# XUANTIE-RV/csi-nn2

Hardware: AMD Instinct MI355X
Metric: mobilenetv1_int8_images_per_sec (higher is better)
Workload: dtype i8; 1 GPU; mobilenetv1 int8 NHWC batch 1/GPU, 28 conv layers in 15 launches, hipGraph replay via csinn_*; ops_per_image=1137480704, algorithmic_bytes_per_image=8323144, algorithmic_bytes_per_image_survey=14444616, parallelism=replicas x1

## Files before the change

### csi-nn2_amd/csrc/stemdw_fused.hip

```cpp
#include <stdio.h>
#include <stdlib.h>

#include "dw_patch.h"

namespace shl {

struct StemDwArgs {
    ConvArgs st;
    ConvArgs dw;
    int32_t bh, bw;
    int32_t tiles_x, tiles_y;
    int32_t rw, npx;
    uint32_t rw_magic, bw_magic;
};

template <int EPQ, int EPD>
__global__ __launch_bounds__(256) void stemdw_fused_kernel(StemDwArgs f)
{
    extern __shared__ __attribute__((aligned(16))) char smem[];
    const ConvArgs &q = f.st;
    const ConvArgs &d = f.dw;
    asm volatile("" ::"s"(q.in), "s"(q.w), "s"(q.acc_init), "s"(q.mult), "s"(q.bias), "s"(q.H), "s"(q.W), "s"(q.Ho), "s"(q.Wo), "s"(q.sh),
                 "s"(q.sw), "s"(q.pt), "s"(q.pl), "s"(q.dh), "s"(q.dw), "s"(q.in_zp));
    asm volatile("" ::"s"(f.bh), "s"(f.bw), "s"(f.tiles_y), "s"(f.rw), "s"(f.npx), "s"(f.rw_magic), "s"(f.bw_magic), "s"(d.N), "s"(d.sh),
                 "s"(d.sw), "s"(d.pt), "s"(d.pl), "s"(d.w), "s"(d.acc_init), "s"(d.mult), "s"(d.bias), "s"(d.out));
    asm volatile("" ::"s"(q.out_zp), "s"(q.out_zp_f), "s"(q.clamp_lo), "s"(q.clamp_hi), "s"(d.out_zp), "s"(d.out_zp_f), "s"(d.clamp_lo),
                 "s"(d.clamp_hi), "s"(d.in_zp), "s"(d.Ho), "s"(d.Wo), "s"(d.H), "s"(d.W), "s"(d.C));
    const int tid = threadIdx.x;
    int32_t *w_lds = reinterpret_cast<int32_t *>(smem);
    int32_t *t_tab = w_lds + 7 * 32;
    uint32_t *patch = reinterpret_cast<uint32_t *>(t_tab + 96);
    if (tid < 224) w_lds[tid] = static_cast<const int32_t *>(q.w)[tid];
    if (tid < 96) {
        const int which = tid >> 5, i = tid & 31;
        t_tab[tid] = which == 0 ? q.acc_init[i] : which == 1 ? __float_as_int(q.mult[i]) : __float_as_int(q.bias[i]);
    }
    const int tx = blockIdx.x;
    int ty = blockIdx.y, n = 0;
    if (d.N > 1) {
        n = ty / f.tiles_y;
        ty -= n * f.tiles_y;
    }
    const int oy0 = ty * f.bh, ox0 = tx * f.bw;
    const int ry0 = oy0 * d.sh - d.pt, rx0 = ox0 * d.sw - d.pl;
    const DwThreadConsts dwk = dw_load_consts(d, 0, tid);

    const int8_t *img = static_cast<const int8_t *>(q.in) + (int64_t)n * q.H * q.W * 3;
    const int ntasks = 2 * f.npx;
    const int ppitch = dw_patch_pitch(f.npx);
    const uint32_t zpad = dw_patch_pad(d);
    for (int base = 0; base < ntasks; base += 256) {
        const bool valid = base + tid < ntasks;
        const int task = valid ? base + tid : ntasks - 1;
        const int j = task >> 1, cb = (task & 1) * 16;
        const int pr = (int)(((uint32_t)j * f.rw_magic) >> 20);
        const int pc = j - pr * f.rw;
        const int sy = ry0 + pr, sx = rx0 + pc;
        const bool inside = (unsigned)sy < (unsigned)q.Ho && (unsigned)sx < (unsigned)q.Wo;
        const int y0 = sy * q.sh - q.pt, x0 = sx * q.sw - q.pl;
        int qv[28];
#pragma unroll
        for (int ky = 0; ky < 3; ++ky)
#pragma unroll
            for (int kx = 0; kx < 3; ++kx) {
                const int y = y0 + ky * q.dh, x = x0 + kx * q.dw;
                const bool ok = inside && (unsigned)y < (unsigned)q.H && (unsigned)x < (unsigned)q.W;
                const int8_t *px = img + ((int64_t)y * q.W + x) * 3;
#pragma unroll
                for (int c = 0; c < 3; ++c) qv[(ky * 3 + kx) * 3 + c] = ok ? (int)px[c] : q.in_zp;
            }
        qv[27] = 0;
        uint32_t q4[7];
#pragma unroll
        for (int g = 0; g < 7; ++g)
            q4[g] = (uint32_t)(qv[4 * g] & 0xFF) | ((uint32_t)(qv[4 * g + 1] & 0xFF) << 8) |
                    ((uint32_t)(qv[4 * g + 2] & 0xFF) << 16) | ((uint32_t)(qv[4 * g + 3] & 0xFF) << 24);
        if (base == 0) __syncthreads();
        int acc[16];
#pragma unroll
        for (int e = 0; e < 16; ++e) acc[e] = 0;
#pragma unroll
        for (int g = 0; g < 7; ++g)
#pragma unroll
            for (int v = 0; v < 4; ++v) {
                const int4 w = *reinterpret_cast<const int4 *>(&w_lds[g * 32 + cb + 4 * v]);
                acc[4 * v + 0] = __builtin_amdgcn_sdot4((int)q4[g], w.x, acc[4 * v + 0], false);
                acc[4 * v + 1] = __builtin_amdgcn_sdot4((int)q4[g], w.y, acc[4 * v + 1], false);
                acc[4 * v + 2] = __builtin_amdgcn_sdot4((int)q4[g], w.z, acc[4 * v + 2], false);
                acc[4 * v + 3] = __builtin_amdgcn_sdot4((int)q4[g], w.w, acc[4 * v + 3], false);
            }
#pragma unroll
        for (int v = 0; v < 4; ++v) {
            const int c = cb + 4 * v;
            const int4 ai = *reinterpret_cast<const int4 *>(t_tab + c);
            const float4 mu = *reinterpret_cast<const float4 *>(t_tab + 32 + c);
            const float4 bi = *reinterpret_cast<const float4 *>(t_tab + 64 + c);
            const uint32_t pk = requant4_i8_sel<EPQ>(acc[4 * v] + ai.x, acc[4 * v + 1] + ai.y, acc[4 * v + 2] + ai.z,
                                               acc[4 * v + 3] + ai.w, mu, bi, q);
            if (valid) patch[dw_patch_slot(j, c >> 2, ppitch)] = inside ? pk : zpad;
        }
    }
    __syncthreads();

    DwPatchGeom g;
    g.bh = f.bh, g.bw = f.bw, g.rw = f.rw, g.bw_magic = f.bw_magic, g.pitch = ppitch;
    g.oy0 = oy0, g.ox0 = ox0, g.ry0 = ry0, g.rx0 = rx0, g.n = n, g.ch0 = 0;
    depthwise_from_patch<EPD>(d, patch, g, dwk, tid, 256);
}

static bool stemdw_geometry(const ConvArgs &q, const ConvArgs &d, StemDwArgs &f)
{
    if (q.Kh != 3 || q.Kw != 3 || q.C != 3 || q.Co != 32) return false;
    if (d.Kh != 3 || d.Kw != 3 || d.dh != 1 || d.dw != 1 || d.C != 32 || d.Co != 32) return false;
    if (d.H != q.Ho || d.W != q.Wo || d.N != q.N || d.sh < 1 || d.sh > 2 || d.sw < 1 || d.sw > 2) return false;
    if (d.pt < 0 || d.pl < 0 || d.pt > 2 || d.pl > 2) return false;
    if ((int64_t)d.Ho * d.Wo * d.C >= ((int64_t)1 << 31)) return false;
    f.bh = d.Ho < 2 ? d.Ho : 2;
    f.bw = d.Wo < 28 ? d.Wo : 28;
    if (const char *e = getenv("SHL_MI355X_STEMDW_TILE")) {
        int h = 0, w = 0;
        if (sscanf(e, "%dx%d", &h, &w) == 2 && h > 0 && w > 0) f.bh = h < d.Ho ? h : d.Ho, f.bw = w < d.Wo ? w : d.Wo;
    }
    f.tiles_y = (d.Ho + f.bh - 1) / f.bh;
    f.tiles_x = (d.Wo + f.bw - 1) / f.bw;
    f.rw = (f.bw - 1) * d.sw + 3;
    f.npx = ((f.bh - 1) * d.sh + 3) * f.rw;
    f.rw_magic = ((1u << 20) + f.rw - 1) / f.rw;
    f.bw_magic = ((1u << 20) + f.bw - 1) / f.bw;
    if (f.npx >= 2048 || f.tiles_x > 65535 || (int64_t)f.tiles_y * d.N > 65535) return false;
    return (int64_t)f.tiles_x * f.tiles_y * d.N <= 2048;
}

bool stemdw_fusable(const ConvArgs &q, const ConvArgs &d)
{
    StemDwArgs f;
    return stemdw_geometry(q, d, f);
}

int launch_stemdw_fused(const ConvArgs &q, const ConvArgs &d, hipStream_t s)
{
    StemDwArgs f;
    f.st = q;
    f.dw = d;
    if (!stemdw_geometry(q, d, f)) {
        set_error("stemdw_fused: the pair does not qualify");
        return SHL_MI355X_ENOTSUP;
    }
    const dim3 grid((unsigned)f.tiles_x, (unsigned)(f.tiles_y * d.N));
    const size_t lds = (size_t)(7 * 32 + 96) * 4 + dw_patch_bytes(f.npx);
    const int epq = (q.act != SHL_MI355X_ACT_NONE && !q.act_clamp) ? -1 : (q.div_exact ? 3 : 0);
    const int epd = (d.act != SHL_MI355X_ACT_NONE && !d.act_clamp) ? -1 : (d.div_exact ? 3 : 0);
    if (epq == 3 && epd == 3) hipLaunchKernelGGL((stemdw_fused_kernel<3, 3>), grid, dim3(256), lds, s, f);
    else if (epq == 0 && epd == 0) hipLaunchKernelGGL((stemdw_fused_kernel<0, 0>), grid, dim3(256), lds, s, f);
    else hipLaunchKernelGGL((stemdw_fused_kernel<-1, -1>), grid, dim3(256), lds, s, f);
    SHL_HIP(hipGetLastError());
    return SHL_MI355X_OK;
}

}
```

Measured before the change: 17470 img/s.

## Compute stem conv with MFMA i8 and buffer-load rows in fused stem+dw kernel

Replaces the per-thread sdot4 stem convolution with a 32x32x32 i8 MFMA per wave. Each lane holds weight fragments and requant constants in registers instead of LDS. Input pixels are fetched as 12-byte buffer loads per kernel row, with byte shifting and masking to apply zero-point padding. The default tile also changes from 2x28 to 4x14. This cuts scalar dot-product work and the LDS weight staging, but adds shift/mask ALU work and new geometry restrictions.

```diff
diff --git a/csi-nn2_amd/csrc/stemdw_fused.hip b/csi-nn2_amd/csrc/stemdw_fused.hip
--- a/csi-nn2_amd/csrc/stemdw_fused.hip
+++ b/csi-nn2_amd/csrc/stemdw_fused.hip
@@ -21,20 +21,12 @@
     const ConvArgs &q = f.st;
     const ConvArgs &d = f.dw;
     asm volatile("" ::"s"(q.in), "s"(q.w), "s"(q.acc_init), "s"(q.mult), "s"(q.bias), "s"(q.H), "s"(q.W), "s"(q.Ho), "s"(q.Wo), "s"(q.sh),
-                 "s"(q.sw), "s"(q.pt), "s"(q.pl), "s"(q.dh), "s"(q.dw), "s"(q.in_zp));
-    asm volatile("" ::"s"(f.bh), "s"(f.bw), "s"(f.tiles_y), "s"(f.rw), "s"(f.npx), "s"(f.rw_magic), "s"(f.bw_magic), "s"(d.N), "s"(d.sh),
-                 "s"(d.sw), "s"(d.pt), "s"(d.pl), "s"(d.w), "s"(d.acc_init), "s"(d.mult), "s"(d.bias), "s"(d.out));
-    asm volatile("" ::"s"(q.out_zp), "s"(q.out_zp_f), "s"(q.clamp_lo), "s"(q.clamp_hi), "s"(d.out_zp), "s"(d.out_zp_f), "s"(d.clamp_lo),
-                 "s"(d.clamp_hi), "s"(d.in_zp), "s"(d.Ho), "s"(d.Wo), "s"(d.H), "s"(d.W), "s"(d.C));
+                 "s"(q.sw), "s"(q.pt), "s"(q.pl), "s"(q.in_zp));
+    asm volatile("" ::"s"(f.bh), "s"(f.bw), "s"(f.tiles_y), "s"(f.rw), "s"(f.npx), "s"(f.rw_magic), "s"(d.N), "s"(d.sh), "s"(d.sw),
+                 "s"(d.pt), "s"(d.pl), "s"(d.w), "s"(d.acc_init), "s"(d.mult), "s"(d.bias));
     const int tid = threadIdx.x;
-    int32_t *w_lds = reinterpret_cast<int32_t *>(smem);
-    int32_t *t_tab = w_lds + 7 * 32;
-    uint32_t *patch = reinterpret_cast<uint32_t *>(t_tab + 96);
-    if (tid < 224) w_lds[tid] = static_cast<const int32_t *>(q.w)[tid];
-    if (tid < 96) {
-        const int which = tid >> 5, i = tid & 31;
-        t_tab[tid] = which == 0 ? q.acc_init[i] : which == 1 ? __float_as_int(q.mult[i]) : __float_as_int(q.bias[i]);
-    }
+    const int lane = tid & 63, frow = lane & 31, khalf = lane >> 5;
+    uint32_t *patch = reinterpret_cast<uint32_t *>(smem);
     const int tx = blockIdx.x;
     int ty = blockIdx.y, n = 0;
     if (d.N > 1) {
@@ -45,59 +37,79 @@
     const int ry0 = oy0 * d.sh - d.pt, rx0 = ox0 * d.sw - d.pl;
     const DwThreadConsts dwk = dw_load_consts(d, 0, tid);
 
-    const int8_t *img = static_cast<const int8_t *>(q.in) + (int64_t)n * q.H * q.W * 3;
-    const int ntasks = 2 * f.npx;
+    const int32_t *w = static_cast<const int32_t *>(q.w) + frow;
+    const int w3 = w[3 * 32];
+    const v4i fa = {w[(4 * khalf + 0) * 32], w[(4 * khalf + 1) * 32], w[(4 * khalf + 2) * 32], khalf ? 0 : w3};
+    v16i ainit;
+    float4 mu[4], bi[4];
+#pragma unroll
+    for (int g = 0; g < 4; ++g) {
+        const int c = 8 * g + 4 * khalf;
+        const int4 ai = *reinterpret_cast<const int4 *>(q.acc_init + c);
+        ainit[4 * g] = ai.x, ainit[4 * g + 1] = ai.y, ainit[4 * g + 2] = ai.z, ainit[4 * g + 3] = ai.w;
+        mu[g] = *reinterpret_cast<const float4 *>(q.mult + c);
+        bi[g] = *reinterpret_cast<const float4 *>(q.bias + c);
+    }
+    const int img_bytes = q.H * q.W * 3;
+    const __amdgpu_buffer_rsrc_t rsrc = __builtin_amdgcn_make_buffer_rsrc(
+        const_cast<int8_t *>(static_cast<const int8_t *>(q.in) + (int64_t)n * img_bytes), 0, img_bytes, 0x00020000);
+    const uint32_t zp4 = (uint32_t)(q.in_zp & 0xff) * 0x01010101u;
     const int ppitch = dw_patch_pitch(f.npx);
     const uint32_t zpad = dw_patch_pad(d);
-    for (int base = 0; base < ntasks; base += 256) {
-        const bool valid = base + tid < ntasks;
-        const int task = valid ? base + tid : ntasks - 1;
-        const int j = task >> 1, cb = (task & 1) * 16;
-        const int pr = (int)(((uint32_t)j * f.rw_magic) >> 20);
-        const int pc = j - pr * f.rw;
-        const int sy = ry0 + pr, sx = rx0 + pc;
+    const int ntiles = (f.npx + 31) >> 5;
+    const int wave = __builtin_amdgcn_readfirstlane(tid >> 6);
+    for (int tile = wave; tile < ntiles; tile += 4) {
+        const int j = tile * 32 + frow;
+        const int jc = j < f.npx ? j : f.npx - 1;
+        const int pr = (int)(((uint32_t)jc * f.rw_magic) >> 20);
+        const int pc = jc - pr * f.rw;
+        int sy = ry0 + pr, sx = rx0 + pc;
         const bool inside = (unsigned)sy < (unsigned)q.Ho && (unsigned)sx < (unsigned)q.Wo;
+        if (!inside) sy = 0, sx = 0;
         const int y0 = sy * q.sh - q.pt, x0 = sx * q.sw - q.pl;
-        int qv[28];
+        uint32_t v[3][3], rows = 0;
+        int shift[3];
 #pragma unroll
-        for (int ky = 0; ky < 3; ++ky)
+        for (int ky = 0; ky < 3; ++ky) {
+            const int y = y0 + ky;
+            const bool yok = (unsigned)y < (unsigned)q.H;
+            rows |= yok ? 0u : 1u << ky;
+            const int off = ((yok ? y : 0) * q.W + x0) * 3;
+            const int offc = off < 0 ? 0 : (off + 12 > img_bytes ? img_bytes - 12 : off);
+            shift[ky] = off - offc;
+            const auto l = __builtin_amdgcn_raw_buffer_load_b96(rsrc, offc, 0, 0);
+            v[ky][0] = l[0], v[ky][1] = l[1], v[ky][2] = l[2];
+        }
+        const uint32_t cols = ((unsigned)x0 >= (unsigned)q.W ? 1u : 0u) | ((unsigned)(x0 + 1) >= (unsigned)q.W ? 2u : 0u) |
+                              ((unsigned)(x0 + 2) >= (unsigned)q.W ? 4u : 0u);
+        const uint32_t m0 = ((cols & 1) ? 0x00FFFFFFu : 0u) | ((cols & 2) ? 0xFF000000u : 0u);
+        const uint32_t m1 = ((cols & 2) ? 0x0000FFFFu : 0u) | ((cols & 4) ? 0xFFFF0000u : 0u);
+        const uint32_t m2 = (cols & 4) ? 0x000000FFu : 0u;
+        uint32_t r[3][3];
 #pragma unroll
-            for (int kx = 0; kx < 3; ++kx) {
-                const int y = y0 + ky * q.dh, x = x0 + kx * q.dw;
-                const bool ok = inside && (unsigned)y < (unsigned)q.H && (unsigned)x < (unsigned)q.W;
-                const int8_t *px = img + ((int64_t)y * q.W + x) * 3;
+        for (int ky = 0; ky < 3; ++ky) {
+            uint32_t v0 = v[ky][0], v1 = v[ky][1], v2 = v[ky][2];
+            if (shift[ky] != 0) {
+                unsigned __int128 x = (unsigned __int128)v0 | (unsigned __int128)v1 << 32 | (unsigned __int128)v2 << 64;
+                x = shift[ky] > 0 ? x >> (8 * shift[ky]) : x << (-8 * shift[ky]);
+                v0 = (uint32_t)x, v1 = (uint32_t)(x >> 32), v2 = (uint32_t)(x >> 64);
+            }
+            const uint32_t ym = (rows >> ky) & 1 ? 0xFFFFFFFFu : 0u;
+            r[ky][0] = ((m0 | ym) & zp4) | (~(m0 | ym) & v0);
+            r[ky][1] = ((m1 | ym) & zp4) | (~(m1 | ym) & v1);
+            r[ky][2] = ((m2 | ym) & zp4) | (~(m2 | ym) & v2);
+        }
+        const int kd2 = (int)((r[0][2] & 0xFFu) | (r[1][0] << 8));
+        const int kd3 = (int)__builtin_amdgcn_alignbyte(r[1][1], r[1][0], 3);
+        const int kd4 = (int)((r[1][1] >> 24) | ((r[1][2] & 0xFFu) << 8) | (r[2][0] << 16));
+        const int kd5 = (int)__builtin_amdgcn_alignbyte(r[2][1], r[2][0], 2);
+        const int kd6 = (int)((r[2][1] >> 16) | ((r[2][2] & 0xFFu) << 16));
+        const v4i fb = khalf ? v4i{kd4, kd5, kd6, 0} : v4i{(int)r[0][0], (int)r[0][1], kd2, kd3};
+        const v16i acc = __builtin_amdgcn_mfma_i32_32x32x32_i8(fa, fb, ainit, 0, 0, 0);
 #pragma unroll
-                for (int c = 0; c < 3; ++c) qv[(ky * 3 + kx) * 3 + c] = ok ? (int)px[c] : q.in_zp;
-            }
-        qv[27] = 0;
-        uint32_t q4[7];
-#pragma unroll
-        for (int g = 0; g < 7; ++g)
-            q4[g] = (uint32_t)(qv[4 * g] & 0xFF) | ((uint32_t)(qv[4 * g + 1] & 0xFF) << 8) |
-                    ((uint32_t)(qv[4 * g + 2] & 0xFF) << 16) | ((uint32_t)(qv[4 * g + 3] & 0xFF) << 24);
-        if (base == 0) __syncthreads();
-        int acc[16];
-#pragma unroll
-        for (int e = 0; e < 16; ++e) acc[e] = 0;
-#pragma unroll
-        for (int g = 0; g < 7; ++g)
-#pragma unroll
-            for (int v = 0; v < 4; ++v) {
-                const int4 w = *reinterpret_cast<const int4 *>(&w_lds[g * 32 + cb + 4 * v]);
-                acc[4 * v + 0] = __builtin_amdgcn_sdot4((int)q4[g], w.x, acc[4 * v + 0], false);
-                acc[4 * v + 1] = __builtin_amdgcn_sdot4((int)q4[g], w.y, acc[4 * v + 1], false);
-                acc[4 * v + 2] = __builtin_amdgcn_sdot4((int)q4[g], w.z, acc[4 * v + 2], false);
-                acc[4 * v + 3] = __builtin_amdgcn_sdot4((int)q4[g], w.w, acc[4 * v + 3], false);
-            }
-#pragma unroll
-        for (int v = 0; v < 4; ++v) {
-            const int c = cb + 4 * v;
-            const int4 ai = *reinterpret_cast<const int4 *>(t_tab + c);
-            const float4 mu = *reinterpret_cast<const float4 *>(t_tab + 32 + c);
-            const float4 bi = *reinterpret_cast<const float4 *>(t_tab + 64 + c);
-            const uint32_t pk = requant4_i8_sel<EPQ>(acc[4 * v] + ai.x, acc[4 * v + 1] + ai.y, acc[4 * v + 2] + ai.z,
-                                               acc[4 * v + 3] + ai.w, mu, bi, q);
-            if (valid) patch[dw_patch_slot(j, c >> 2, ppitch)] = inside ? pk : zpad;
+        for (int g = 0; g < 4; ++g) {
+            const uint32_t pk = requant4_i8_sel<EPQ>(acc[4 * g], acc[4 * g + 1], acc[4 * g + 2], acc[4 * g + 3], mu[g], bi[g], q);
+            if (j < f.npx) patch[dw_patch_slot(j, 2 * g + khalf, ppitch)] = inside ? pk : zpad;
         }
     }
     __syncthreads();
@@ -111,12 +123,14 @@
 static bool stemdw_geometry(const ConvArgs &q, const ConvArgs &d, StemDwArgs &f)
 {
     if (q.Kh != 3 || q.Kw != 3 || q.C != 3 || q.Co != 32) return false;
+    if (q.dh != 1 || q.dw != 1 || q.pl < 0 || q.pl > 2 || (q.Wo - 1) * q.sw + 3 - q.W - q.pl > 2) return false;
+    if ((int64_t)q.H * q.W * 3 < 12 || (int64_t)q.H * q.W * 3 >= ((int64_t)1 << 31)) return false;
     if (d.Kh != 3 || d.Kw != 3 || d.dh != 1 || d.dw != 1 || d.C != 32 || d.Co != 32) return false;
     if (d.H != q.Ho || d.W != q.Wo || d.N != q.N || d.sh < 1 || d.sh > 2 || d.sw < 1 || d.sw > 2) return false;
     if (d.pt < 0 || d.pl < 0 || d.pt > 2 || d.pl > 2) return false;
     if ((int64_t)d.Ho * d.Wo * d.C >= ((int64_t)1 << 31)) return false;
-    f.bh = d.Ho < 2 ? d.Ho : 2;
-    f.bw = d.Wo < 28 ? d.Wo : 28;
+    f.bh = d.Ho < 4 ? d.Ho : 4;
+    f.bw = d.Wo < 14 ? d.Wo : 14;
     if (const char *e = getenv("SHL_MI355X_STEMDW_TILE")) {
         int h = 0, w = 0;
         if (sscanf(e, "%dx%d", &h, &w) == 2 && h > 0 && w > 0) f.bh = h < d.Ho ? h : d.Ho, f.bw = w < d.Wo ? w : d.Wo;
@@ -147,7 +161,7 @@
         return SHL_MI355X_ENOTSUP;
     }
     const dim3 grid((unsigned)f.tiles_x, (unsigned)(f.tiles_y * d.N));
-    const size_t lds = (size_t)(7 * 32 + 96) * 4 + dw_patch_bytes(f.npx);
+    const size_t lds = dw_patch_bytes(f.npx);
     const int epq = (q.act != SHL_MI355X_ACT_NONE && !q.act_clamp) ? -1 : (q.div_exact ? 3 : 0);
     const int epd = (d.act != SHL_MI355X_ACT_NONE && !d.act_clamp) ? -1 : (d.div_exact ? 3 : 0);
     if (epq == 3 && epd == 3) hipLaunchKernelGGL((stemdw_fused_kernel<3, 3>), grid, dim3(256), lds, s, f);
```

Result: no change. 17420 img/s, median of 3 (-0.3%).
